# millardjn/rusty_sr

Measured on AMD Instinct MI355X. Metric: output megapixels/sec at 3x upscale (BASELINE '4x'; reference factor is hard-wired 3), higher is better.
Workload: dtype f32

## Files before the change

### rusty_sr_amd/csrc/sr_api.cpp

```cpp
#include <hip/hip_runtime.h>

#include <algorithm>
#include <cmath>
#include <cstdio>
#include <cstdlib>
#include <chrono>
#include <cstring>
#include <new>
#include <string>
#include <thread>
#include <vector>

#include "../../include/srhip.h"
#include "../../include/srhip_experimental.h"
#include "sr_kernels.h"
#include "sr_internal.h"

namespace {

struct ParamLayout {
    size_t conv0, f_bias, f_activ, exp_bias, l_bias[3], l_activ[3], conv1, conv2, conv3, conv5, conv6, conv7, conv8,
        conv9, conv10, end;
    int E;
    explicit ParamLayout(int f) {
// ... 317 lines not shown
        pack_conv0_split(w, params + L.conv0);
        c->off_w0h = push(w);
        for (int split = 0; split < 2; ++split) {
            auto ident = [](int, int j) { return j; };
            auto expand = [&](int nt, int j) { return split ? expand_channel_t(factor, nt, j) : expand_channel(factor, nt, j); };
            const bool h16 = split != 0;
            auto conv = [&](const float* wp, int ks) { if (h16) pack_steps_h16(w, wp, ks); else pack_steps(w, wp, ks, 1, split != 0, ident); };
            auto exp3 = [&](const float* wp) { pack_steps(w, wp, 3, expand_tiles(factor), split != 0, expand); };
            size_t* off = split ? c->off_wh : c->off_w;
            w.clear(); conv(params + L.conv1, 5);
            off[1] = push(w);
            w.clear(); conv(params + L.conv2, 5); conv(params + L.conv5, 3);
            off[2] = push(w);
            w.clear(); conv(params + L.conv3, 5); conv(params + L.conv6, 3); conv(params + L.conv8, 3);
            off[3] = push(w);
            w.clear();
            exp3(params + L.conv7); exp3(params + L.conv9); exp3(params + L.conv10);
            if (split) pack_lin_split(w, factor);
            else pack_lin(w, factor);
            off[4] = push(w);
        }
        w.clear(); pack_steps_wino(w, params + L.conv1);
        c->off_wino1 = push(w);
        const size_t boff[4] = {L.f_bias, L.l_bias[0], L.l_bias[1], L.l_bias[2]};
        const size_t aoff[4] = {L.f_activ, L.l_activ[0], L.l_activ[1], L.l_activ[2]};
        for (int s = 0; s < 4; ++s) c->off_bias[s] = push(vec32(boff[s], 32));
        for (int s = 0; s < 4; ++s) c->off_beta[s] = push(vec32(aoff[s], 32));
        {
            std::vector<float> eb((size_t)expand_tiles(factor) * 32, 0.0f);
            for (int nt = 0; nt < expand_tiles(factor); ++nt)
                for (int j = 0; j < 32; ++j) {
                    const int ch = expand_channel(factor, nt, j);
                    if (ch >= 0) eb[nt * 32 + j] = params[L.exp_bias + ch];
                }
            c->off_bias[4] = push(eb);
        }
        for (size_t k = L.conv1; k < L.end && c->split_ok; ++k) c->split_ok = std::fabs(params[k]) < 65504.0f;
        for (size_t k = L.conv0; k < L.conv0 + 2400 && c->split_ok; ++k) c->split_ok = std::fabs(params[k]) < 65504.0f;
        mark("weight packing (host)");
        HIPCHK(c, hipHostMalloc((void**)&c->h_domain, 64, hipHostMallocMapped));
        *c->h_domain = 0;
        HIPCHK(c, hipHostGetDevicePointer((void**)&c->d_domain, c->h_domain, 0));
        for (auto& w : c->ws) HIPCHK(c, hipMalloc((void**)&w.d_queue, 5 * 8 * sizeof(int)));

        HIPCHK(c, hipMalloc((void**)&c->d_params, host.size() * sizeof(float)));
        mark("hipMalloc x3");
// ... 74 lines not shown
        while (*v) {
            c->env_rows.push_back(atoi(v));
            while (*v && *v != ',') ++v;
            if (*v) ++v;
        }
    } else if (!strcmp(key, "geo")) {
        c->env_geo = strcmp(v, "0") != 0;
    } else if (!strcmp(key, "tail")) {
        c->env_tail = *v ? (float)atof(v) : -1.0f;
    } else if (!strcmp(key, "fork")) {
        c->env_fork = *v ? atoi(v) : -1;
    } else if (!strcmp(key, "forkshare")) {
        c->fork_share = *v ? std::min(0.9, std::max(0.1, atof(v))) : 0.5;
    } else if (!strcmp(key, "forkmin")) {
        c->fork_min_rounds = *v ? atof(v) : 3.5;
    } else if (!strcmp(key, "forktune")) {
        c->fork_autotune = strcmp(v, "0") != 0;
        sr_device_guard restore_device;
        (void)hipSetDevice(c->device);
        sr_fork_tune_clear(c);
    } else if (!strcmp(key, "halo")) {
        c->layer_halos = !strcmp(v, "layers");
    } else if (!strcmp(key, "wino")) {
        c->wino = strcmp(v, "0") != 0;
    } else if (!strcmp(key, "bw")) {
        c->env_bw = *v ? atoi(v) : -1;
    } else {
        return SR_E_INVALID;
    }
    return SR_OK;
}

int sr_get_experiment(sr_ctx* c, const char* key, char* buf, size_t cap) {
    if (!c || !key || !buf || cap == 0) return SR_E_INVALID;
    std::string out;
    if (!strcmp(key, "forktune")) {
        char line[160];
        for (const auto& t : c->fork_tune) {
            snprintf(line, sizeof line, "%dx%d+%d+%d %s %s %s %.4f %.4f\n", t.H, t.W, t.top, t.bot, t.precision == SR_PRECISION_F32 ? "f32" : "split_f16",
                     t.img_u8 ? "u8" : "f32", t.decided < 0 ? "measuring" : (t.decided ? "forked" : "undivided"),
                     t.best[0] < 1e29f ? t.best[0] : 0.f, t.best[1] < 1e29f ? t.best[1] : 0.f);
            out += line;
        }
    } else if (!strcmp(key, "plan")) {
        for (const auto& r : c->plan_rec) out += r.first + (r.second > 1 ? " x" + std::to_string(r.second) : std::string()) + "\n";
    } else {
        return SR_E_INVALID;
// ... 105 lines not shown
    bool mark = false;
    hipStream_t s = nullptr;
    struct Launch { int y0, y1, ty8, ty4, th, grid; bool pipe; } L[5];
    float* feat[4] = {nullptr, nullptr, nullptr, nullptr};
    int prepare();
    int launch(int st) const;
};

int StackJob::prepare() {
    static const int margin[5] = {5, 3, 2, 1, 0};
    tiles_x = (W + 31) / 32;
    const int rc = ensure_features(c, *ws, n, H, W, tiles_x, s);
    if (rc != SR_OK) return rc;
    const int cus = c->cus > 0 ? c->cus : 256;
    const int resident = 2 * cus;
    const bool planar = c->precision == SR_PRECISION_SPLIT_F16;
    for (int k = 0; k < 4; ++k) feat[k] = ws->d_feat[k] + (planar ? (size_t)kFeatPad * ws->pitch * 32 + kFeatPad * 4 : ((size_t)kFeatPad * ws->pitch + kFeatPad) * 32);
    for (int st = 0; st < 5; ++st) {
        Launch& l = L[st];
        l.y0 = layers ? top : std::max(0, top - margin[st]);
        l.y1 = layers ? bot : std::min(H, bot + margin[st]);
        const int rows = l.y1 - l.y0;
        const long tiles8 = (long)n * tiles_x * ((rows + 7) / 8);
        const bool wino8 = st == 1 && c->precision == SR_PRECISION_F32 && c->wino;
        const int forced = (st == 4 && c->factor == 4 && c->precision == SR_PRECISION_SPLIT_F16) ? 4 : c->env_th[st];
        const bool small_launch = tiles8 < 2L * resident;
        const bool split = c->precision == SR_PRECISION_SPLIT_F16;
        const bool one_small_round = small_launch && (long)n * tiles_x * ((rows + 3) / 4) <= resident;
        l.pipe = st > 0 && c->env_pipe != 0 && (c->env_pipe == 2 || !small_launch || split || (st >= 2 && one_small_round));
        l.ty8 = (rows + 7) / 8; l.ty4 = 0;
        if (forced == 4 || (!forced && small_launch && !wino8 && (!split || tiles8 < cus))) {
            l.ty8 = 0; l.ty4 = (rows + 3) / 4;
        } else if (!forced && l.pipe && !small_launch) {
            const double rounds = (double)tiles8 / resident;
            float tail = c->env_tail;
            if (tail < 0.0f) tail = (!split && rounds >= 3.0 && !forked && st != 4) ? 1.0f : 0.0f;
            if (tail > 0.0f) {
                const long per_row = (long)n * tiles_x;
                const int want = (int)((tail * resident + per_row - 1) / per_row);
                l.ty8 = std::max(0, (rows - 4 * want) / 8);
                l.ty4 = std::max(0, (rows - 8 * l.ty8 + 3) / 4);
            }
        }
        if (!forced && l.pipe && !small_launch && !split && l.ty4 == 0 && (double)tiles8 / resident >= 3.0 && rows % 8 >= 1 && rows % 8 <= 4) {
            l.ty8 = rows / 8; l.ty4 = 1;
        }
        if (l.ty8 > 0 && l.ty4 > 0 && (long)n * tiles_x * (l.ty8 + l.ty4) <= resident) {
            l.ty8 = 0; l.ty4 = (rows + 3) / 4;
        }
        l.th = l.ty8 > 0 ? 8 : 4;
        if (!l.pipe && l.ty8 > 0) { l.ty8 = (rows + 7) / 8; l.ty4 = 0; }
        const int ntiles = n * tiles_x * (l.ty8 + l.ty4);
        l.grid = l.pipe ? std::min(ntiles, resident) : ntiles;
    }
    return SR_OK;
}

int StackJob::launch(int st) const {
    const int cus = c->cus > 0 ? c->cus : 256;
// ... 25 lines not shown
            HIPCHK(c, sr_launch_conv0(a, l.th, c->precision, std::min(a.n_tiles, 8 * cus), img_u8, s));
            return SR_OK;
        };
        if (!gate || !gate->ready) return rows(y0, y1);
        const int lo = late_top > 0 ? std::max(y0, late_top + 2) : y0, hi = late_bot > 0 ? std::min(y1, H - late_bot - 2) : y1;
        int rc = lo < hi ? rows(lo, hi) : SR_OK;
        if (rc != SR_OK) return rc;
        if (mark && gate->mark[0]) HIPCHK(c, hipEventRecord(gate->mark[0], s));
        HIPCHK(c, hipStreamWaitEvent(s, gate->ready, 0));
        if (mark && gate->mark[1]) HIPCHK(c, hipEventRecord(gate->mark[1], s));
        if (lo >= hi) return rows(y0, y1);
        rc = rows(y0, lo);
        return rc != SR_OK ? rc : rows(hi, y1);
    }
    StageArgs a{};
    float* f = feat[0]; float* l1 = feat[1]; float* l2 = feat[2]; float* l3 = feat[3];
    a.pitch = ws->pitch; a.img_stride = ws->img_stride;
    switch (st) {
        case 1: a.src[0] = f; a.dst = l1; break;
        case 2: a.src[0] = f; a.src[1] = l1; a.dst = l2; break;
        case 3: a.src[0] = f; a.src[1] = l1; a.src[2] = l2; a.dst = l3; break;
        case 4: a.src[0] = l1; a.src[1] = l2; a.src[2] = l3; a.img = d_img; a.out = d_out; break;
    }
    const bool wino = st == 1 && c->precision == SR_PRECISION_F32 && c->wino;
    a.wpack = P + (c->precision ? c->off_wh[st] : wino ? c->off_wino1 : c->off_w[st]); a.bias = P + c->off_bias[st];
    a.beta = st < 4 ? P + c->off_beta[st] : nullptr;
    a.H = H; a.W = W; a.img_ch = img_ch;
    a.y_begin = y0; a.y_end = y1; a.tiles_x = tiles_x;
    a.n_img = n; a.queue = ws->d_queue + st * 8; a.domain = c->d_domain;
    a.grid[0] = make_tile_grid(8, y0, l.ty8, tiles_x, n, bw);
    a.grid[1] = make_tile_grid(4, y0 + 8 * l.ty8, l.ty4, tiles_x, n, bw);
    if (l.pipe) HIPCHK(c, sr_launch_stage_pipe(st, c->factor, a, c->precision, l.grid, img_u8, out_u8, wino, s));
    else HIPCHK(c, sr_launch_stage(st, c->factor, a, l.th, c->precision, l.grid, img_u8, out_u8, wino, s));
    return SR_OK;
}

}

int sr_run_stack(sr_ctx* c, const void* d_img, bool img_u8, int img_ch, int n, int H, int W, int halo_top,
                 int halo_bot, void* d_out, bool out_u8, hipStream_t s, int slot, const sr_halo_gate* gate) {
    if (!c || !d_img || !d_out || slot < 0 || slot > 1) return SR_E_INVALID;
    sr_device_guard restore_device;
    if (n <= 0 || H <= 0 || W <= 0) return SR_E_INVALID;
    if (img_u8 && img_ch != 3 && img_ch != 4) return SR_E_INVALID;
    if (c->graph != SR_GRAPH_SR_NET) {
        if (halo_top || halo_bot || gate) return SR_E_INVALID;
        if (c->graph == SR_GRAPH_DOWNSAMPLE && (H < 3 || W < 3)) return SR_E_INVALID;
        if (img_u8 != out_u8) return SR_E_INVALID;
// ... 744 lines not shown
```

### rusty_sr_amd/csrc/sr_internal.h

```cpp
#pragma once
#include <hip/hip_runtime.h>

#include <cstdint>
#include <string>
#include <utility>
#include <vector>

#include "../../include/srhip.h"

struct sr_ctx {
    int device = 0;
    int cus = 0, clock_mhz = 0;
    char name[128] = {0};
    hipStream_t stream = nullptr;
    float* d_params = nullptr;
    void* d_qtab = nullptr;
    size_t off_w0 = 0, off_w0h = 0, off_w[5] = {0}, off_wh[5] = {0}, off_bias[5] = {0}, off_beta[5] = {0};
    size_t off_wino1 = 0;
    bool wino = true;
    int precision = 0;
    bool split_ok = true;
    int* h_domain = nullptr;
    int* d_domain = nullptr;
    int domain_fallbacks = 0;
    bool dev_fault = false;
    int graph = SR_GRAPH_SR_NET;
    int factor = SR_FACTOR;
    struct Workspace {
        float* d_feat[4] = {nullptr, nullptr, nullptr, nullptr};
        size_t feat_cap_px = 0;
        int geo_n = 0, geo_h = 0, geo_w = 0;
        int pitch = 0; long img_stride = 0;
        int* d_queue = nullptr;
    } ws[2];
    hipStream_t stream2 = nullptr;
    void* d_in[2] = {nullptr, nullptr};  size_t in_cap[2] = {0, 0};
    void* d_out[2] = {nullptr, nullptr}; size_t out_cap[2] = {0, 0};
    hipStream_t copy_out = nullptr;
    hipStream_t copy_in = nullptr;
    int pipelined_calls = 0;
    std::vector<hipEvent_t> pool;
    int pipeline = 1;
// ... 145 lines not shown
```

### rusty_sr_amd/csrc/sr_kernels.hip

```cpp
#include <hip/hip_runtime.h>
#include <stddef.h>
#include <stdint.h>

#include <mutex>
#include <set>
#include <type_traits>
#include <utility>

#include "sr_kernels.h"

#pragma clang fp contract(off)

typedef float f32x2 __attribute__((ext_vector_type(2)));
struct f32p { float x, y; };
__device__ __forceinline__ f32p operator+(f32p a, f32p b) { return f32p{a.x + b.x, a.y + b.y}; }
__device__ __forceinline__ f32p operator-(f32p a, f32p b) { return f32p{a.x - b.x, a.y - b.y}; }
__device__ __forceinline__ f32p operator*(f32p a, f32p b) { return f32p{a.x * b.x, a.y * b.y}; }
__device__ __forceinline__ f32p p_fma(f32p a, f32p b, f32p c) { return f32p{__builtin_fmaf(a.x, b.x, c.x), __builtin_fmaf(a.y, b.y, c.y)}; }
__device__ __forceinline__ void store_map8(char* p, uint32_t a, uint32_t b) { *(uint2*)p = make_uint2(a, b); }
typedef float f32x4 __attribute__((ext_vector_type(4)));
typedef float f32x16 __attribute__((ext_vector_type(16)));
typedef _Float16 f16x8 __attribute__((ext_vector_type(8)));
typedef _Float16 f16x2 __attribute__((ext_vector_type(2)));

// ... 510 lines not shown
        __builtin_amdgcn_sched_barrier(0);
        cur = nxt;
      }
    }
}

constexpr int kWinoGroups = 5 * 7 * 2;
constexpr int kWinoSteps = (kWinoGroups + 3) / 4;
constexpr int wino_acc(int k) { return k < 4 ? k : k - 3; }
constexpr int wino_ca(int k) { return k == 0 ? 0 : k == 1 ? 1 : k == 2 ? 2 : k == 3 ? 1 : k == 4 ? 3 : k == 5 ? 4 : 3; }
constexpr int wino_cb(int k) { return k == 0 ? 2 : k == 1 ? 2 : k == 2 ? 1 : k == 3 ? 3 : k == 4 ? 4 : k == 5 ? 3 : 5; }
constexpr bool wino_add(int k) { return k == 1 || k == 4; }

template <bool ADD>
__device__ __forceinline__ void wino_u4(f32x2 x0, f32x2 y0, f32x2 x1, f32x2 y1, f32x2& u0, f32x2& u1) {
    if constexpr (ADD)
        asm("v_pk_add_f32 %0, %2, %3\n\tv_pk_add_f32 %1, %4, %5\n\ts_nop 1"
            : "=&v"(u0), "=&v"(u1) : "v"(x0), "v"(y0), "v"(x1), "v"(y1));
    else
        asm("v_pk_add_f32 %0, %2, %3 neg_lo:[0,1] neg_hi:[0,1]\n\tv_pk_add_f32 %1, %4, %5 neg_lo:[0,1] neg_hi:[0,1]\n\ts_nop 1"
            : "=&v"(u0), "=&v"(u1) : "v"(x0), "v"(y0), "v"(x1), "v"(y1));
}

template <int TWH, int PS, int T, typename Stream>
__device__ __forceinline__ void half_steps_wino(f32x16 (&acc)[4], const char* hb, const char* ring, Stream& sm, int wave, int lane) {
    static_assert(TWH >= kTW + 4, "a pair reads six pixels from its first halo column on");
    const int i = lane & 31, h = lane >> 5;
    const int wlane = (h * 32 + i) * 16;
    const int row = wave * T + (T == 2 ? i >> 4 : 0);
    const char* abase = hb + h * PS + (row * TWH + 2 * (i & 15)) * 16;
    struct Ops { f32x4 x, y, b; };
    auto load = [&](Ops& o, int g, int sl) {
        const int rr = g & 1, k = (g >> 1) % 7, ky = (g >> 1) / 7;
        const char* ab = abase + rr * 2 * PS + ky * TWH * 16;
        o.b = *(const f32x4*)(ring + sl * 4096 + wlane + (g & 3) * 1024);
        o.x = *(const f32x4*)(ab + wino_ca(k) * 16);
        o.y = *(const f32x4*)(ab + wino_cb(k) * 16);
    };
    auto mfma = [&](const Ops& o, int g) {
        const int k = (g >> 1) % 7;
        const f32x2 x0 = {o.x[0], o.x[1]}, x1 = {o.x[2], o.x[3]}, y0 = {o.y[0], o.y[1]}, y1 = {o.y[2], o.y[3]};
        f32x2 u0, u1;
        if (wino_add(k)) wino_u4<true>(x0, y0, x1, y1, u0, u1);
        else wino_u4<false>(x0, y0, x1, y1, u0, u1);
        const float u[4] = {u0.x, u0.y, u1.x, u1.y};
#pragma unroll
        for (int e = 0; e < 4; ++e) acc[wino_acc(k)] = __builtin_amdgcn_mfma_f32_32x32x2f32(u[e], o.b[e], acc[wino_acc(k)], 0, 0, 0);
    };
    Ops cur, nxt;
    load(cur, 0, sm.slot());
#pragma unroll
    for (int s = 0; s < kWinoSteps; ++s) {
        const int ngroups = kWinoGroups - 4 * s < 4 ? kWinoGroups - 4 * s : 4;
        sm.begin_step();
#pragma unroll
        for (int q = 0; q < 3; ++q) {
            if (q + 1 < ngroups) {
                load(nxt, 4 * s + q + 1, sm.slot());
                sm.piece(4 * s + q);
                __builtin_amdgcn_sched_barrier(0);
                mfma(cur, 4 * s + q);
                __builtin_amdgcn_sched_barrier(0);
                cur = nxt;
            }
        }
        const bool last = s == kWinoSteps - 1;
        sm.template end_step<0>(last);
        if (!last) load(nxt, 4 * s + 4, sm.slot());
        sm.piece(4 * s + 3);
        __builtin_amdgcn_sched_barrier(0);
        mfma(cur, 4 * s + ngroups - 1);
        __builtin_amdgcn_sched_barrier(0);
        cur = nxt;
    }
}

template <int TWH, int PS, int LO, int KS, int T, int NTN, typename Stream>
__device__ __forceinline__ void half_steps_h(f32x16 (&accm)[NTN * T], f32x16 (&accx)[NTN * T], const char* hb, const char* ring,
                                             Stream& sm, int wave, int lane) {
    constexpr int NT = KS * KS, NP = (NT + 1) / 2;
    const int i = lane & 31, h = lane >> 5;
    const int wlane = (h * 32 + i) * 16;
    const char* abase = hb + h * PS + ((wave * T) * TWH + i) * 16;
    struct Ops { f16x8 bh[2], bl[2], ah[2][T], al[2][T]; };
    auto row_id = [](int p, int ts, int m) {
        const int t = 2 * p + ts;
        return t < NT ? (t / KS) * 16 + (t % KS) + m : -1;
    };
    auto load = [&](Ops& o, const Ops& prev, int pp, int p, int sl) {
        const char* wb = ring + sl * 4096 + wlane;
#pragma unroll
        for (int ts = 0; ts < 2; ++ts) {
            const int t = 2 * p + ts;
            if (t >= NT) continue;
// ... 414 lines not shown
                    };
                    if (full_x) {
                        uint32_t px[16];
#pragma unroll
                        for (int r = 0; r < 16; r += 2) quant2(r, px[r], px[r + 1]);
                        if (writer) for_each_acc_row([&](int r, int row) { base[row * FACTOR] = px[r]; });
                    } else {
#pragma unroll
                        for (int r = 0; r < 16; r += 2) {
                            uint32_t p0, p1;
                            quant2(r, p0, p1);
                            const int row0 = (r & 3) + 8 * (r >> 2);
                            if (writer && x0 + 4 * h + row0 < a.W) base[row0 * FACTOR] = p0;
                            if (writer && x0 + 4 * h + row0 + 1 < a.W) base[(row0 + 1) * FACTOR] = p1;
                        }
                    }
                }
            }
        }
    }
    return stores;
}

template <int T>
__device__ __forceinline__ int stage_epilogue_wino(const StageArgs& a, const f32x16 (&acc)[4], float bias, float beta, int n, int x0, int y0,
                                                   int wave, int lane, float* stage_lds) {
    const int i = lane & 31, h = lane >> 5;
    const bool full_x = x0 + kTW <= a.W;
    int stores = 0;
#pragma unroll
    for (int m = 0; m < T; ++m) {
        const int y = y0 + wave * T + m;
        if (y >= a.y_end) continue;
        float* grow = a.dst + ((size_t)n * a.img_stride + (long)y * a.pitch + x0) * 32;
        float o[16];
#pragma unroll
        for (int k = 0; k < 8; k += 2) {
            const int r = 8 * m + k;
            const f32x2 m0 = {acc[0][r], acc[0][r + 1]}, m1 = {acc[1][r], acc[1][r + 1]};
            const f32x2 m2 = {acc[2][r], acc[2][r + 1]}, m3 = {acc[3][r], acc[3][r + 1]};
            const f32x2 bb = {bias, bias};
            const f32x2 p0 = belu2(((m0 + m1) + m2) + bb, beta), p1 = belu2(((m1 - m2) - m3) + bb, beta);
            o[2 * k] = p0.x; o[2 * k + 1] = p1.x; o[2 * k + 2] = p0.y; o[2 * k + 3] = p1.y;
        }
        auto pixel = [&](int v) { return 2 * (((v >> 1) & 3) + 8 * (v >> 3) + 4 * h) + (v & 1); };
        if (full_x && stage_lds) {
            float* sp = stage_lds + i;
#pragma unroll
            for (int v = 0; v < 16; ++v) sp[pixel(v) * 32] = o[v];
            const f32x4* lp = (const f32x4*)stage_lds + lane;
            const f32x4 v0 = lp[0], v1 = lp[64], v2 = lp[128], v3 = lp[192];
            f32x4* gp = (f32x4*)grow + lane;
            gp[0] = v0; gp[64] = v1; gp[128] = v2; gp[192] = v3;
            stores += 4;
        } else if (full_x) {
#pragma unroll
            for (int v = 0; v < 16; ++v) grow[pixel(v) * 32 + i] = o[v];
            stores += 16;
        } else {
#pragma unroll
            for (int v = 0; v < 16; ++v)
                if (x0 + pixel(v) < a.W) grow[pixel(v) * 32 + i] = o[v];
        }
    }
    return stores;
// ... 187 lines not shown

__device__ __forceinline__ void run_of_xcd(int x, int ntiles, int& start, int& count) {
    const int q = ntiles >> 3, r = ntiles & 7;
    count = q + (x < r ? 1 : 0);
    start = x < r ? x * (q + 1) : r * (q + 1) + (x - r) * q;
}
__device__ __forceinline__ int queue_slot(int x, int nbig, int nsmall, int idx) {
    int start, count;
    run_of_xcd(x, nbig, start, count);
    if (idx < count) return start + idx;
    idx -= count;
    run_of_xcd(x, nsmall, start, count);
    return idx < count ? nbig + start + idx : -1;
}
__device__ __forceinline__ int queue_total(int x, int nbig, int nsmall) {
    int start, cb, cs;
    run_of_xcd(x, nbig, start, cb);
    run_of_xcd(x, nsmall, start, cs);
    return cb + cs;
}
__device__ __forceinline__ int queue_first(int block, int nbig, int nsmall) { return queue_slot(block & 7, nbig, nsmall, block >> 3); }
template <int TH, int NSRC, int KS0, bool FINAL, bool IMG_U8, bool OUT_U8, int PREC, int FACTOR = 3, bool WINO = false>
__global__ __launch_bounds__(256, 2) void conv_stage_kernel(StageArgs a) {
    static_assert(!WINO || (NSRC == 1 && KS0 == 5 && !FINAL && PREC == 0), "WINO: stage 1 of the exact mode");
    __builtin_amdgcn_s_setprio(3);
    constexpr int NW = 4, T = TH / NW;
    constexpr int NTN = FINAL ? (FACTOR * FACTOR + 9) / 10 : 1;
    using G0 = TileGeom<TH, KS0>;
    extern __shared__ __attribute__((aligned(16))) char smem[];
    char* tile = smem;
    char* ring = smem + 8 * G0::PLANE;

    const int tid = threadIdx.x, lane = tid & 63;
    const int wave = __builtin_amdgcn_readfirstlane(tid >> 6);
    const int i = lane & 31;
    constexpr bool H16 = kH16<PREC, FINAL>;
    constexpr int NTAPS = WINO ? 2 * kWinoSteps
                        : H16 ? KS0 * KS0 + (NSRC - 1) * 9
                              : 2 * ((KS0 * KS0 + 1) / 2 + (NSRC - 1) * 5) * NTN;
    const TileGrid& grid = a.grid[TH == 8 ? 0 : 1];
    float bias[NTN];
#pragma unroll
    for (int nt = 0; nt < NTN; ++nt) bias[nt] = a.bias[nt * 32 + i];
    const float beta = FINAL ? 0.f : a.beta[i];

    TileOffsets<TH, KS0, NW> off0;
    TileOffsets<TH, 3, NW> off3;
    off0.template init<PREC>(a.pitch, wave, lane);
    if constexpr (NSRC >= 2) off3.template init<PREC>(a.pitch, wave, lane);
    int n, tx, ty;
    tile_coords(grid, a.tiles_x, xcd_remap(blockIdx.x, gridDim.x), n, tx, ty);
    const int x0 = tx * kTW, y0 = grid.y0 + ty * TH;
#pragma unroll
    for (int k = 0; k < kRingAhead; ++k) weight_chunk_async(ring + k * 4096, a.wpack + k * kChunkFloats, wave, lane);
    stage_tile<TH, KS0, PREC, NW>(tile, a.src[0], off0, a.img_stride, a.pitch, n, y0, x0, wave, lane);

    f32x16 acc[NTN * T], accx[PREC == 1 ? NTN * T : 1];
#pragma unroll
    for (int m = 0; m < NTN * T; ++m)
#pragma unroll
        for (int r = 0; r < 16; ++r) {
            acc[m][r] = (PREC == 1 && !FINAL) ? bias[0] : 0.f;
            if constexpr (PREC == 1) accx[m][r] = 0.f;
        }
    f32x4 qm[H16 ? T : 1][2][2], qx[H16 ? T : 1][2][2];
    f32x4 bias2[2], beta2[2];
    if constexpr (H16) {
#pragma unroll
        for (int ch = 0; ch < 2; ++ch) {
            bias2[ch] = *(const f32x4*)(a.bias + 16 * ch + 4 * (lane >> 4));
            beta2[ch] = *(const f32x4*)(a.beta + 16 * ch + 4 * (lane >> 4));
        }
#pragma unroll
        for (int m = 0; m < T; ++m)
#pragma unroll
            for (int k = 0; k < 4; ++k) { qm[m][k >> 1][k & 1] = bias2[k & 1]; qx[m][k >> 1][k & 1] = f32x4{0.f, 0.f, 0.f, 0.f}; }
    }
    f32x16 wacc[WINO ? 4 : 1];
#pragma unroll
    for (int p = 0; p < (WINO ? 4 : 1); ++p)
#pragma unroll
        for (int r = 0; r < 16; ++r) wacc[p][r] = 0.f;
    int gtap = 0, slot = 0;
    auto taps = [&](auto ks_tag) {
        constexpr int KS = decltype(ks_tag)::value;
        if constexpr (WINO) {
            using G = TileGeom<TH, KS>;
            RingStream sm{ring, a.wpack, gtap, slot, NTAPS, wave, lane};
#pragma unroll 1
            for (int half = 0; half < 2; ++half) half_steps_wino<G::TWH, G::PLANE, T>(wacc, tile + half * 4 * G::PLANE, ring, sm, wave, lane);
        } else if constexpr (H16) source_steps_h16<TH, KS, T>(qm, qx, tile, ring, a.wpack, gtap, slot, NTAPS, wave, lane);
        else source_steps<TH, KS, T, NTN, PREC>(acc, accx, tile, ring, a.wpack, gtap, slot, NTAPS, wave, lane);
    };
    ring_barrier<0>();
    __builtin_amdgcn_s_setprio(0);
    taps(std::integral_constant<int, KS0>{});
    if constexpr (NSRC >= 2) {
        __builtin_amdgcn_s_setprio(3);
        stage_tile<TH, 3, PREC, NW>(tile, a.src[1], off3, a.img_stride, a.pitch, n, y0, x0, wave, lane);
        ring_barrier<0>();
        __builtin_amdgcn_s_setprio(0);
        taps(std::integral_constant<int, 3>{});
    }
    if constexpr (NSRC >= 3) {
        __builtin_amdgcn_s_setprio(3);
        stage_tile<TH, 3, PREC, NW>(tile, a.src[2], off3, a.img_stride, a.pitch, n, y0, x0, wave, lane);
        ring_barrier<0>();
        __builtin_amdgcn_s_setprio(0);
        taps(std::integral_constant<int, 3>{});
    }
    __builtin_amdgcn_s_setprio(3);
    if constexpr (FINAL)
        lin_taps<TH, T, IMG_U8, NW * 64, NTN, PREC, FACTOR>(acc, accx, tile, ring, a, a.wpack + (size_t)NTAPS * kChunkFloats, n, y0, x0, wave, lane, tid);
    uint32_t dom = 0;
    if constexpr (WINO) {
        stage_epilogue_wino<T>(a, wacc, bias[0], beta, n, x0, y0, wave, lane, nullptr);
    } else if constexpr (H16) {
        stage_epilogue_h16<T>(a, qm, qx, beta2, n, x0, y0, wave, lane, dom);
    } else if constexpr (FINAL && PREC == 1) {
        f32x4 fbias[NTN][4];
#pragma unroll
        for (int nt = 0; nt < NTN; ++nt)
#pragma unroll
            for (int k = 0; k < 4; ++k) fbias[nt][k] = *(const f32x4*)(a.bias + 32 * nt + 16 * (lane >> 5) + 4 * k);
        stage_epilogue_final_t<T, NTN, OUT_U8, FACTOR>(a, acc, accx, fbias, n, x0, y0, wave, lane);
    } else {
        static_assert(PREC == 0, "the split-half mode's tiles have epilogues of their own");
        stage_epilogue<TH, T, NTN, FINAL, OUT_U8, FACTOR>(a, acc, bias, beta, n, x0, y0, wave, lane);
    }
    if constexpr (PREC == 1 && !FINAL) domain_report(dom, a.domain);
}

#define SR_WAIT_ROW(k, extra) "s_waitcnt vmcnt(" #k ")" extra "\n\ts_branch .Lsrwait%=\n\t"
#define SR_WAIT_ROWS10(b, extra)                                                                                              \
    SR_WAIT_ROW(b##0, extra) SR_WAIT_ROW(b##1, extra) SR_WAIT_ROW(b##2, extra) SR_WAIT_ROW(b##3, extra) SR_WAIT_ROW(b##4, extra) \
    SR_WAIT_ROW(b##5, extra) SR_WAIT_ROW(b##6, extra) SR_WAIT_ROW(b##7, extra) SR_WAIT_ROW(b##8, extra) SR_WAIT_ROW(b##9, extra)
#define SR_WAIT_JUMP(maxn)                                                                                                   \
    "s_max_i32 %0, %1, 0\n\ts_min_i32 %0, %0, " #maxn "\n\ts_lshl_b32 %0, %0, 3\n\ts_add_u32 %0, %0, 12\n\t"                 \
    "s_getpc_b64 vcc\n\ts_add_u32 vcc_lo, vcc_lo, %0\n\ts_addc_u32 vcc_hi, vcc_hi, 0\n\ts_setpc_b64 vcc\n\t"
// ... 247 lines not shown
    int step_no;
    Hook last_step_hook;
    __device__ __forceinline__ void begin_step() {
        step_request(st, gs0 + step_no, ring_lds, wbase, lane);
        if (mailbox && step_no == snap_step) queue_presolve(a, xcd, wave, lane, st, qs);
        ++step_no;
    }
    __device__ __forceinline__ void piece(int g) {
        if (g < HalfTile<KSN>::G::NG && g < rq.ng) {
            htn.stage_one(g, rq.origin, rq.dst);
            st.tile_seq = ++st.issued;
        }
    }
    __device__ __forceinline__ int slot() const { return st.slot; }
    template <int EXTRA> __device__ __forceinline__ void end_step(bool last) {
        if (last) last_step_hook();
        if (last && mailbox) queue_publish(a, xcd, wave, lane, st, qs, mailbox);
        step_advance<EXTRA>(st, last, PREC == 1 && gs0 + step_no <= kRingAhead);
    }
};

template <int NSRC, int KS0, bool FINAL, bool IMG_U8, bool OUT_U8, int PREC, int FACTOR = 3, bool WINO = false>
__global__ __launch_bounds__(256, 2) void conv_stage_pipe_kernel(StageArgs a) {
    static_assert(!WINO || (NSRC == 1 && KS0 == 5 && !FINAL && PREC == 0), "WINO: stage 1 of the exact mode");
    __builtin_amdgcn_s_setprio(3);
    constexpr int NTN = FINAL ? (FACTOR * FACTOR + 9) / 10 : 1;
    using H0 = HalfTile<KS0>;
    using H3 = HalfTile<3>;
    constexpr int HB = H0::BYTES;
    constexpr int NH = 2 * NSRC;
    constexpr bool H16 = kH16<PREC, FINAL>;
    constexpr int NSTEPS = WINO ? 2 * kWinoSteps
                         : H16 ? KS0 * KS0 + (NSRC - 1) * 9
                               : 2 * (H0::STEPS + (NSRC - 1) * H3::STEPS) * NTN;
    extern __shared__ __attribute__((aligned(16))) char smem[];
    char* ring = smem + 2 * HB;
    volatile int* s_next = (volatile int*)(ring + kRingBytes);
    float* s_wlin = (float*)(ring + kRingBytes + 16);
    float* s_lut = s_wlin + 9 * NTN * 128;
    constexpr bool kLinOwn = FINAL && NTN == 1;
    float* s_xown = s_lut + 256;
    const uint32_t lds0 = lds_addr(smem);

    const int tid = threadIdx.x, lane = tid & 63;
    const int wave = __builtin_amdgcn_readfirstlane(tid >> 6);
    const int i = lane & 31;
    const int nbig = a.grid[0].ntiles, nsmall = a.grid[1].ntiles;
    const int xcd = blockIdx.x & 7;
    const uint32_t ring_lds = __builtin_amdgcn_readfirstlane(lds_addr(ring) + wave * 1024);
    const char* wbase = uniform_ptr((const char*)a.wpack + wave * 1024);
    float bias[NTN];
#pragma unroll
    for (int nt = 0; nt < NTN; ++nt) bias[nt] = a.bias[nt * 32 + i];
    const float beta = FINAL ? 0.f : a.beta[i];
    f32x4 bias2[2], beta2[2];
// ... 70 lines not shown
        f32x16 acc[NTN * T], accx[PREC == 1 ? NTN * T : 1];
#pragma unroll
        for (int m = 0; m < NTN * T; ++m)
#pragma unroll
            for (int r = 0; r < 16; ++r) {
                acc[m][r] = (PREC == 1 && !FINAL) ? bias[0] : 0.f;
                if constexpr (PREC == 1) accx[m][r] = 0.f;
            }
        f32x4 qm[H16 ? T : 1][2][2], qx[H16 ? T : 1][2][2];
        if constexpr (H16) {
#pragma unroll
            for (int m = 0; m < T; ++m)
#pragma unroll
                for (int k = 0; k < 4; ++k) { qm[m][k >> 1][k & 1] = bias2[k & 1]; qx[m][k >> 1][k & 1] = f32x4{0.f, 0.f, 0.f, 0.f}; }
        }
        constexpr bool QUAD = FINAL && PREC == 0 && T == 2;
        QuadAcc qa[QUAD ? NTN : 1];
        if constexpr (QUAD) {
#pragma unroll
            for (int nt = 0; nt < NTN; ++nt)
#pragma unroll
                for (int g = 0; g < 8; ++g) qa[nt][g] = f32x4{0.f, 0.f, 0.f, 0.f};
        }
        f32x16 wacc[WINO ? 4 : 1];
#pragma unroll
        for (int p = 0; p < (WINO ? 4 : 1); ++p)
#pragma unroll
            for (int r = 0; r < 16; ++r) wacc[p][r] = 0.f;
        QueueState qs{0u, 0u, 0, 0, -1};
        if (!single) queue_pull_async(a, xcd, wave, lane, st, qs);
        st.have_next = false;
        LinPrefetch<IMG_U8, TH> linpx;
        auto do_half = [&](auto jc) {
            constexpr int j = decltype(jc)::value;
            constexpr int src = j >> 1;
            constexpr int KSJ = src == 0 ? KS0 : 3;
            constexpr int KSN = (j + 1 < NH) ? (((j + 1) >> 1) == 0 ? KS0 : 3) : KS0;
            const uint32_t other = lds0 + ((j + 1) & 1) * HB;
            const char* hb = smem + (j & 1) * HB;
            if constexpr (j == 1) {
                const int next = single ? -1 : __builtin_amdgcn_readfirstlane(*s_next);
                st.have_next = next >= 0;
                if (st.have_next) coords(next, nn, nx0, ny0, nsmall_tile);
            }
            HalfRequest rq;
            if constexpr (j + 1 < NH)
                rq = HalfRequest{T == 2 ? HalfTile<KSN>::G::NG : HalfTile<KSN>::NG_SMALL,
                                 HalfTile<KSN>::template origin_of<PREC>(a.src[(j + 1) >> 1], (j + 1) & 1, a.img_stride, a.pitch, n, y0, x0, wave),
                                 HalfTile<KSN>::plane_of(other, wave)};
            else
                rq = HalfRequest{!st.have_next ? 0 : nsmall_tile ? HalfTile<KSN>::NG_SMALL : HalfTile<KSN>::G::NG,
                                 HalfTile<KSN>::template origin_of<PREC>(a.src[0], 0, a.img_stride, a.pitch, nn, ny0, nx0, wave),
                                 HalfTile<KSN>::plane_of(other, wave)};
            if constexpr (FINAL && j == (kLinOwn ? NH - 2 : NH - 1)) linpx.issue(a, n, y0, x0, tid, st);
            const HalfTile<KSN>* htn;
            if constexpr (KSN == KS0) htn = (const HalfTile<KSN>*)&h0; else htn = (const HalfTile<KSN>*)&h3;
            using GJ = TileGeom<8, KSJ>;
            constexpr int PAIRS_J = (KSJ * KSJ - 1) / 2;
            constexpr int STEPS_J = WINO ? kWinoSteps : H16 ? PAIRS_J + (j & 1) : HalfTile<KSJ>::STEPS * NTN;
            constexpr int GS0 = WINO ? j * kWinoSteps : H16 ? (src == 0 ? 0 : KS0 * KS0 + (src - 1) * 9) + (j & 1) * PAIRS_J
                                    : (j == 0 ? 0 : j == 1 ? H0::STEPS : 2 * H0::STEPS + (j - 2) * H3::STEPS) * NTN;
            constexpr int LIN_LO_J = LinPrefetch<IMG_U8, TH>::NPIX * 8;
            auto lin_store = [&]() {
                if constexpr (kLinOwn && j == NH - 2) {
                    if constexpr (PREC == 1) linpx.store_split((char*)s_xown, LIN_LO_J, (const uint32_t*)s_lut, 4.0f * FACTOR * FACTOR, tid, st);
                    else linpx.store(s_xown, s_lut, tid, st);
                    asm volatile("s_waitcnt lgkmcnt(0)" ::: "memory");
                }
            };
            PipeStream<PREC, KSN, decltype(lin_store)> sm{st, rq, *htn, a, ring_lds, wbase, GS0, wave, lane, (j == 0 && !single) ? s_next : nullptr, xcd, qs, STEPS_J > 3 ? STEPS_J - 3 : 0, 0, lin_store};
            if constexpr (WINO) half_steps_wino<GJ::TWH, GJ::PLANE, T>(wacc, hb, ring, sm, wave, lane);
            else if constexpr (QUAD) half_steps_f32<GJ::TWH, GJ::PLANE, KSJ, T, NTN, true, FACTOR>(qa, hb, ring, sm, wave, lane);
            else if constexpr (PREC == 0) half_steps_f32<GJ::TWH, GJ::PLANE, KSJ, T, NTN>(acc, hb, ring, sm, wave, lane);
            else if constexpr (H16) half_steps_h16<GJ::TWH, GJ::PLANE, 2, KSJ, T, (j & 1) != 0, -HB>(qm, qx, hb, ring, sm, wave, lane);
            else half_steps_h<GJ::TWH, GJ::PLANE, 2, KSJ, T, NTN>(acc, accx, hb, ring, sm, wave, lane);
        };
        do_half(std::integral_constant<int, 0>{});
        do_half(std::integral_constant<int, 1>{});
        if constexpr (NH > 2) { do_half(std::integral_constant<int, 2>{}); do_half(std::integral_constant<int, 3>{}); }
        if constexpr (NH > 4) { do_half(std::integral_constant<int, 4>{}); do_half(std::integral_constant<int, 5>{}); }
        if constexpr (FINAL) {
            constexpr int LIN_LO = LinPrefetch<IMG_U8, TH>::NPIX * 8;
            float* s_x = kLinOwn ? s_xown : (float*)(smem + HB);
            if constexpr (!kLinOwn) {
                if constexpr (PREC == 1) linpx.store_split((char*)s_x, LIN_LO, (const uint32_t*)s_lut, 4.0f * FACTOR * FACTOR, tid, st);
                else linpx.store(s_x, s_lut, tid, st);
                asm volatile("s_waitcnt lgkmcnt(0)" ::: "memory");
                __builtin_amdgcn_s_barrier();
                asm volatile("" ::: "memory");
            }
            if constexpr (PREC == 1) lin_mfma_h<TH, T, NTN>(acc, accx, (const char*)s_x, LIN_LO, (const f16x8*)s_wlin, wave, lane);
            else if constexpr (QUAD) lin_mfma_quad<NTN, FACTOR>(qa, s_x, s_wlin, wave, lane);
            else lin_mfma<TH, T, NTN>(acc, s_x, s_wlin, wave, lane);
            if constexpr (!kLinOwn) {
                asm volatile("s_waitcnt lgkmcnt(0)" ::: "memory");
                __builtin_amdgcn_s_barrier();
                asm volatile("" ::: "memory");
            }
        }
        int stores;
        if constexpr (H16) stores = stage_epilogue_h16<T>(a, qm, qx, beta2, n, x0, y0, wave, lane, dom);
        else if constexpr (QUAD) stores = stage_epilogue_quad<NTN, OUT_U8, FACTOR>(a, qa, qbias, n, x0, y0, wave, lane);
        else if constexpr (kFinalT) stores = stage_epilogue_final_t<T, NTN, OUT_U8, FACTOR>(a, acc, accx, fbias, n, x0, y0, wave, lane);
        else {
            float* scratch = FINAL ? nullptr : (float*)(smem + ((NH - 1) & 1) * HB + wave * H0::G::PLANE);
            if constexpr (WINO) stores = stage_epilogue_wino<T>(a, wacc, bias[0], beta, n, x0, y0, wave, lane, scratch);
            else stores = stage_epilogue<TH, T, NTN, FINAL, OUT_U8, FACTOR>(a, acc, bias, beta, n, x0, y0, wave, lane, scratch);
        }
        if constexpr (PREC == 1) st.issued += stores;
    };

    constexpr bool kBigTiles = !(FINAL && FACTOR == 4 && PREC == 1);
    int budget = nbig + nsmall;
    while (true) {
        if constexpr (kBigTiles) {
            if (small) tile_body(std::integral_constant<int, 1>{});
            else tile_body(std::integral_constant<int, 2>{});
        } else {
            if (!small) __builtin_trap();
            tile_body(std::integral_constant<int, 1>{});
        }
        if (!st.have_next) break;
        if (--budget <= 0) {
            asm volatile("s_waitcnt vmcnt(0)" ::: "memory");
            __builtin_trap();
        }
        n = nn; x0 = nx0; y0 = ny0; small = nsmall_tile;
    }
    if constexpr (PREC == 1 && !FINAL) domain_report(dom, a.domain);
// ... 68 lines not shown
    hipError_t e = hipGetDevice(&dev);
    if (e != hipSuccess) return e;
    {
        std::lock_guard<std::mutex> lock(mu);
        const auto key = std::make_pair((const void*)kern, dev);
        if (!configured.count(key)) {
            e = hipFuncSetAttribute((const void*)kern, hipFuncAttributeMaxDynamicSharedMemorySize, (int)lds);
            if (e != hipSuccess) return e;
            configured.insert(key);
        }
    }
    hipLaunchKernelGGL(kern, dim3(nblk), dim3(kThreads), lds, s, a);
    return hipGetLastError();
}

template <int TH, int PREC>
static hipError_t launch_stage_t(int stage, int factor, const StageArgs& a, int nblk, bool img_u8, bool out_u8, bool wino,
                                 hipStream_t s) {
    switch (stage) {
        case 1:
            if constexpr (PREC == 0)
                if (wino) return launch_with_lds(conv_stage_kernel<TH, 1, 5, false, false, false, 0, 3, true>, a, nblk, stage_lds_bytes<TH, 5>(), s);
            return launch_with_lds(conv_stage_kernel<TH, 1, 5, false, false, false, PREC>, a, nblk, stage_lds_bytes<TH, 5>(), s);
        case 2: return launch_with_lds(conv_stage_kernel<TH, 2, 5, false, false, false, PREC>, a, nblk, stage_lds_bytes<TH, 5>(), s);
        case 3: return launch_with_lds(conv_stage_kernel<TH, 3, 5, false, false, false, PREC>, a, nblk, stage_lds_bytes<TH, 5>(), s);
        case 4:
#define SR_FINAL(F)                                                                                                          \
            if (img_u8 && out_u8) return launch_with_lds(conv_stage_kernel<TH, 3, 3, true, true, true, PREC, F>, a, nblk, stage_lds_bytes<TH, 3>(), s); \
            if (!img_u8 && !out_u8) return launch_with_lds(conv_stage_kernel<TH, 3, 3, true, false, false, PREC, F>, a, nblk, stage_lds_bytes<TH, 3>(), s); \
            return hipErrorInvalidValue;
            if (factor == 3) { SR_FINAL(3) }
            if (factor == 2) { SR_FINAL(2) }
            if (factor == 4) { SR_FINAL(4) }
#undef SR_FINAL
            return hipErrorInvalidValue;
        default: return hipErrorInvalidValue;
    }
}

template <int PREC>
static hipError_t launch_stage_pipe_t(int stage, int factor, const StageArgs& a, int grid, bool img_u8, bool out_u8, bool wino, hipStream_t s) {
    constexpr size_t lds5 = 2 * (size_t)HalfTile<5>::BYTES + kRingBytes + 16;
    constexpr size_t lds3_1 = 2 * (size_t)HalfTile<3>::BYTES + kRingBytes + 16 + 9 * 128 * sizeof(float) + 256 * sizeof(float) + 10 * 34 * 16;
    constexpr size_t lds3_2 = 2 * (size_t)HalfTile<3>::BYTES + kRingBytes + 16 + 9 * 2 * 128 * sizeof(float) + 256 * sizeof(float);
    static_assert(lds3_1 <= 80 * 1024 && lds3_2 <= 80 * 1024, "two workgroups per CU");
    const size_t lds3 = factor == 4 ? lds3_2 : lds3_1;
    switch (stage) {
        case 1:
            if constexpr (PREC == 0)
                if (wino) return launch_with_lds(conv_stage_pipe_kernel<1, 5, false, false, false, 0, 3, true>, a, grid, lds5, s);
            return launch_with_lds(conv_stage_pipe_kernel<1, 5, false, false, false, PREC>, a, grid, lds5, s);
        case 2: return launch_with_lds(conv_stage_pipe_kernel<2, 5, false, false, false, PREC>, a, grid, lds5, s);
        case 3: return launch_with_lds(conv_stage_pipe_kernel<3, 5, false, false, false, PREC>, a, grid, lds5, s);
        case 4:
#define SR_FINAL(F)                                                                                                          \
            if (img_u8 && out_u8) return launch_with_lds(conv_stage_pipe_kernel<3, 3, true, true, true, PREC, F>, a, grid, lds3, s); \
            if (!img_u8 && !out_u8) return launch_with_lds(conv_stage_pipe_kernel<3, 3, true, false, false, PREC, F>, a, grid, lds3, s); \
            return hipErrorInvalidValue;
            if (factor == 3) { SR_FINAL(3) }
            if (factor == 2) { SR_FINAL(2) }
            if (factor == 4) { SR_FINAL(4) }
#undef SR_FINAL
            return hipErrorInvalidValue;
    }
    return hipErrorInvalidValue;
}
hipError_t sr_launch_stage_pipe(int stage, int factor, const StageArgs& a, int prec, int grid, bool img_u8, bool out_u8, bool wino, hipStream_t s) {
    return prec == 0 ? launch_stage_pipe_t<0>(stage, factor, a, grid, img_u8, out_u8, wino, s)
                     : launch_stage_pipe_t<1>(stage, factor, a, grid, img_u8, out_u8, wino, s);
}

hipError_t sr_launch_stage(int stage, int factor, const StageArgs& a, int th, int prec, int nblk, bool img_u8,
                           bool out_u8, bool wino, hipStream_t s) {
    if (prec == 0)
        return th == 8 ? launch_stage_t<8, 0>(stage, factor, a, nblk, img_u8, out_u8, wino, s)
// ... 5 lines not shown
```

Before: 5017.

## Extend Winograd-style path to stage 2 with a pairwise 3x3 source

Extends the Winograd-style exact f32 convolution path, previously used only for stage 1, to stage 2. The 5x5 source uses the existing Winograd steps, and the second 3x3 source uses a new pairwise-tap MFMA routine that accumulates into a fifth accumulator, which is folded into the odd-pixel output during the epilogue. The goal is fewer MFMA and weight-streaming steps for stage 2. The cost is more accumulator registers, a new weight pack, and turning off the tail split for this stage. The wino setting becomes an integer that defaults to enabling both stages.

```diff
diff --git a/rusty_sr_amd/csrc/sr_api.cpp b/rusty_sr_amd/csrc/sr_api.cpp
--- a/rusty_sr_amd/csrc/sr_api.cpp
+++ b/rusty_sr_amd/csrc/sr_api.cpp
@@ -363,6 +363,8 @@
         }
         w.clear(); pack_steps_wino(w, params + L.conv1);
         c->off_wino1 = push(w);
+        w.clear(); pack_steps_wino(w, params + L.conv2); pack_steps(w, params + L.conv5, 3, 1, false, [](int, int j) { return j; });
+        c->off_wino2 = push(w);
         const size_t boff[4] = {L.f_bias, L.l_bias[0], L.l_bias[1], L.l_bias[2]};
         const size_t aoff[4] = {L.f_activ, L.l_activ[0], L.l_activ[1], L.l_activ[2]};
         for (int s = 0; s < 4; ++s) c->off_bias[s] = push(vec32(boff[s], 32));
@@ -483,7 +485,7 @@
     } else if (!strcmp(key, "halo")) {
         c->layer_halos = !strcmp(v, "layers");
     } else if (!strcmp(key, "wino")) {
-        c->wino = strcmp(v, "0") != 0;
+        c->wino = !strcmp(v, "0") ? 0 : !strcmp(v, "1") ? 1 : 2;
     } else if (!strcmp(key, "bw")) {
         c->env_bw = *v ? atoi(v) : -1;
     } else {
@@ -635,7 +637,7 @@
         l.y1 = layers ? bot : std::min(H, bot + margin[st]);
         const int rows = l.y1 - l.y0;
         const long tiles8 = (long)n * tiles_x * ((rows + 7) / 8);
-        const bool wino8 = st == 1 && c->precision == SR_PRECISION_F32 && c->wino;
+        const bool wino8 = c->precision == SR_PRECISION_F32 && (st == 1 || st == 2) && st <= c->wino;
         const int forced = (st == 4 && c->factor == 4 && c->precision == SR_PRECISION_SPLIT_F16) ? 4 : c->env_th[st];
         const bool small_launch = tiles8 < 2L * resident;
         const bool split = c->precision == SR_PRECISION_SPLIT_F16;
@@ -647,7 +649,7 @@
         } else if (!forced && l.pipe && !small_launch) {
             const double rounds = (double)tiles8 / resident;
             float tail = c->env_tail;
-            if (tail < 0.0f) tail = (!split && rounds >= 3.0 && !forked && st != 4) ? 1.0f : 0.0f;
+            if (tail < 0.0f) tail = (!split && rounds >= 3.0 && !forked && st != 4 && !(st == 2 && wino8)) ? 1.0f : 0.0f;
             if (tail > 0.0f) {
                 const long per_row = (long)n * tiles_x;
                 const int want = (int)((tail * resident + per_row - 1) / per_row);
@@ -719,8 +721,8 @@
         case 3: a.src[0] = f; a.src[1] = l1; a.src[2] = l2; a.dst = l3; break;
         case 4: a.src[0] = l1; a.src[1] = l2; a.src[2] = l3; a.img = d_img; a.out = d_out; break;
     }
-    const bool wino = st == 1 && c->precision == SR_PRECISION_F32 && c->wino;
-    a.wpack = P + (c->precision ? c->off_wh[st] : wino ? c->off_wino1 : c->off_w[st]); a.bias = P + c->off_bias[st];
+    const bool wino = c->precision == SR_PRECISION_F32 && (st == 1 || st == 2) && st <= c->wino;
+    a.wpack = P + (c->precision ? c->off_wh[st] : !wino ? c->off_w[st] : st == 1 ? c->off_wino1 : c->off_wino2); a.bias = P + c->off_bias[st];
     a.beta = st < 4 ? P + c->off_beta[st] : nullptr;
     a.H = H; a.W = W; a.img_ch = img_ch;
     a.y_begin = y0; a.y_end = y1; a.tiles_x = tiles_x;
diff --git a/rusty_sr_amd/csrc/sr_internal.h b/rusty_sr_amd/csrc/sr_internal.h
--- a/rusty_sr_amd/csrc/sr_internal.h
+++ b/rusty_sr_amd/csrc/sr_internal.h
@@ -17,7 +17,8 @@
     void* d_qtab = nullptr;
     size_t off_w0 = 0, off_w0h = 0, off_w[5] = {0}, off_wh[5] = {0}, off_bias[5] = {0}, off_beta[5] = {0};
     size_t off_wino1 = 0;
-    bool wino = true;
+    size_t off_wino2 = 0;
+    int wino = 2;
     int precision = 0;
     bool split_ok = true;
     int* h_domain = nullptr;
diff --git a/rusty_sr_amd/csrc/sr_kernels.hip b/rusty_sr_amd/csrc/sr_kernels.hip
--- a/rusty_sr_amd/csrc/sr_kernels.hip
+++ b/rusty_sr_amd/csrc/sr_kernels.hip
@@ -556,8 +556,8 @@
             : "=&v"(u0), "=&v"(u1) : "v"(x0), "v"(y0), "v"(x1), "v"(y1));
 }
 
-template <int TWH, int PS, int T, typename Stream>
-__device__ __forceinline__ void half_steps_wino(f32x16 (&acc)[4], const char* hb, const char* ring, Stream& sm, int wave, int lane) {
+template <int TWH, int PS, int T, int NA, typename Stream>
+__device__ __forceinline__ void half_steps_wino(f32x16 (&acc)[NA], const char* hb, const char* ring, Stream& sm, int wave, int lane) {
     static_assert(TWH >= kTW + 4, "a pair reads six pixels from its first halo column on");
     const int i = lane & 31, h = lane >> 5;
     const int wlane = (h * 32 + i) * 16;
@@ -604,6 +604,57 @@
         sm.piece(4 * s + 3);
         __builtin_amdgcn_sched_barrier(0);
         mfma(cur, 4 * s + ngroups - 1);
+        __builtin_amdgcn_sched_barrier(0);
+        cur = nxt;
+    }
+}
+
+template <int TWH, int PS, int T, typename Stream>
+__device__ __forceinline__ void half_steps_pairs(f32x16 (&acc)[5], const char* hb, const char* ring, Stream& sm, int wave, int lane) {
+    constexpr int NT = 9, NP = (NT + 1) / 2;
+    static_assert(TWH >= kTW + 2, "a pair reads four pixels from its first halo column on");
+    const int i = lane & 31, h = lane >> 5;
+    const int wlane = (h * 32 + i) * 16;
+    const int row = wave * T + (T == 2 ? i >> 4 : 0);
+    const char* abase = hb + h * PS + (row * TWH + 2 * (i & 15)) * 16;
+    struct Ops { f32x4 x, y, b; };
+    auto load = [&](Ops& o, int p, int q, int sl) {
+        const int t = 2 * p + (q >> 1), ky = t / 3, kx = t - ky * 3;
+        const char* ab = abase + (q & 1) * 2 * PS + (ky * TWH + kx) * 16;
+        o.b = *(const f32x4*)(ring + sl * 4096 + wlane + q * 1024);
+        o.x = *(const f32x4*)ab;
+        o.y = *(const f32x4*)(ab + 16);
+    };
+    auto mfma = [&](const Ops& o) {
+#pragma unroll
+        for (int e = 0; e < 4; ++e) {
+            acc[0] = __builtin_amdgcn_mfma_f32_32x32x2f32(o.x[e], o.b[e], acc[0], 0, 0, 0);
+            acc[4] = __builtin_amdgcn_mfma_f32_32x32x2f32(o.y[e], o.b[e], acc[4], 0, 0, 0);
+        }
+    };
+    Ops cur, nxt;
+    load(cur, 0, 0, sm.slot());
+#pragma unroll
+    for (int p = 0; p < NP; ++p) {
+        const int ngroups = (2 * p + 1 < NT) ? 4 : 2;
+        sm.begin_step();
+#pragma unroll
+        for (int q = 0; q < 3; ++q) {
+            if (q + 1 < ngroups) {
+                load(nxt, p, q + 1, sm.slot());
+                sm.piece(4 * p + q);
+                __builtin_amdgcn_sched_barrier(0);
+                mfma(cur);
+                __builtin_amdgcn_sched_barrier(0);
+                cur = nxt;
+            }
+        }
+        const bool last = p == NP - 1;
+        sm.template end_step<0>(last);
+        if (!last) load(nxt, p + 1, 0, sm.slot());
+        sm.piece(4 * p + 3);
+        __builtin_amdgcn_sched_barrier(0);
+        mfma(cur);
         __builtin_amdgcn_sched_barrier(0);
         cur = nxt;
     }
@@ -1064,9 +1115,10 @@
     return stores;
 }
 
-template <int T>
-__device__ __forceinline__ int stage_epilogue_wino(const StageArgs& a, const f32x16 (&acc)[4], float bias, float beta, int n, int x0, int y0,
+template <int T, int NA>
+__device__ __forceinline__ int stage_epilogue_wino(const StageArgs& a, const f32x16 (&acc)[NA], float bias, float beta, int n, int x0, int y0,
                                                    int wave, int lane, float* stage_lds) {
+    static_assert(NA == 4 || NA == 5, "four position sets, or four and stage 2's odd-pixel set");
     const int i = lane & 31, h = lane >> 5;
     const bool full_x = x0 + kTW <= a.W;
     int stores = 0;
@@ -1082,7 +1134,9 @@
             const f32x2 m0 = {acc[0][r], acc[0][r + 1]}, m1 = {acc[1][r], acc[1][r + 1]};
             const f32x2 m2 = {acc[2][r], acc[2][r + 1]}, m3 = {acc[3][r], acc[3][r + 1]};
             const f32x2 bb = {bias, bias};
-            const f32x2 p0 = belu2(((m0 + m1) + m2) + bb, beta), p1 = belu2(((m1 - m2) - m3) + bb, beta);
+            f32x2 y1 = (m1 - m2) - m3;
+            if constexpr (NA == 5) y1 = y1 + f32x2{acc[4][r], acc[4][r + 1]};
+            const f32x2 p0 = belu2(((m0 + m1) + m2) + bb, beta), p1 = belu2(y1 + bb, beta);
             o[2 * k] = p0.x; o[2 * k + 1] = p1.x; o[2 * k + 2] = p0.y; o[2 * k + 3] = p1.y;
         }
         auto pixel = [&](int v) { return 2 * (((v >> 1) & 3) + 8 * (v >> 3) + 4 * h) + (v & 1); };
@@ -1316,7 +1370,7 @@
 __device__ __forceinline__ int queue_first(int block, int nbig, int nsmall) { return queue_slot(block & 7, nbig, nsmall, block >> 3); }
 template <int TH, int NSRC, int KS0, bool FINAL, bool IMG_U8, bool OUT_U8, int PREC, int FACTOR = 3, bool WINO = false>
 __global__ __launch_bounds__(256, 2) void conv_stage_kernel(StageArgs a) {
-    static_assert(!WINO || (NSRC == 1 && KS0 == 5 && !FINAL && PREC == 0), "WINO: stage 1 of the exact mode");
+    static_assert(!WINO || (NSRC <= 2 && KS0 == 5 && !FINAL && PREC == 0), "WINO: stages 1 and 2 of the exact mode");
     __builtin_amdgcn_s_setprio(3);
     constexpr int NW = 4, T = TH / NW;
     constexpr int NTN = FINAL ? (FACTOR * FACTOR + 9) / 10 : 1;
@@ -1329,7 +1383,7 @@
     const int wave = __builtin_amdgcn_readfirstlane(tid >> 6);
     const int i = lane & 31;
     constexpr bool H16 = kH16<PREC, FINAL>;
-    constexpr int NTAPS = WINO ? 2 * kWinoSteps
+    constexpr int NTAPS = WINO ? 2 * (kWinoSteps + (NSRC - 1) * 5)
                         : H16 ? KS0 * KS0 + (NSRC - 1) * 9
                               : 2 * ((KS0 * KS0 + 1) / 2 + (NSRC - 1) * 5) * NTN;
     const TileGrid& grid = a.grid[TH == 8 ? 0 : 1];
@@ -1370,9 +1424,10 @@
 #pragma unroll
             for (int k = 0; k < 4; ++k) { qm[m][k >> 1][k & 1] = bias2[k & 1]; qx[m][k >> 1][k & 1] = f32x4{0.f, 0.f, 0.f, 0.f}; }
     }
-    f32x16 wacc[WINO ? 4 : 1];
-#pragma unroll
-    for (int p = 0; p < (WINO ? 4 : 1); ++p)
+    constexpr int NWACC = WINO ? 3 + NSRC : 1;
+    f32x16 wacc[NWACC];
+#pragma unroll
+    for (int p = 0; p < NWACC; ++p)
 #pragma unroll
         for (int r = 0; r < 16; ++r) wacc[p][r] = 0.f;
     int gtap = 0, slot = 0;
@@ -1382,7 +1437,10 @@
             using G = TileGeom<TH, KS>;
             RingStream sm{ring, a.wpack, gtap, slot, NTAPS, wave, lane};
 #pragma unroll 1
-            for (int half = 0; half < 2; ++half) half_steps_wino<G::TWH, G::PLANE, T>(wacc, tile + half * 4 * G::PLANE, ring, sm, wave, lane);
+            for (int half = 0; half < 2; ++half) {
+                if constexpr (KS == KS0) half_steps_wino<G::TWH, G::PLANE, T>(wacc, tile + half * 4 * G::PLANE, ring, sm, wave, lane);
+                else half_steps_pairs<G::TWH, G::PLANE, T>(wacc, tile + half * 4 * G::PLANE, ring, sm, wave, lane);
+            }
         } else if constexpr (H16) source_steps_h16<TH, KS, T>(qm, qx, tile, ring, a.wpack, gtap, slot, NTAPS, wave, lane);
         else source_steps<TH, KS, T, NTN, PREC>(acc, accx, tile, ring, a.wpack, gtap, slot, NTAPS, wave, lane);
     };
@@ -1408,7 +1466,7 @@
         lin_taps<TH, T, IMG_U8, NW * 64, NTN, PREC, FACTOR>(acc, accx, tile, ring, a, a.wpack + (size_t)NTAPS * kChunkFloats, n, y0, x0, wave, lane, tid);
     uint32_t dom = 0;
     if constexpr (WINO) {
-        stage_epilogue_wino<T>(a, wacc, bias[0], beta, n, x0, y0, wave, lane, nullptr);
+        stage_epilogue_wino<T, NWACC>(a, wacc, bias[0], beta, n, x0, y0, wave, lane, nullptr);
     } else if constexpr (H16) {
         stage_epilogue_h16<T>(a, qm, qx, beta2, n, x0, y0, wave, lane, dom);
     } else if constexpr (FINAL && PREC == 1) {
@@ -1702,7 +1760,7 @@
 
 template <int NSRC, int KS0, bool FINAL, bool IMG_U8, bool OUT_U8, int PREC, int FACTOR = 3, bool WINO = false>
 __global__ __launch_bounds__(256, 2) void conv_stage_pipe_kernel(StageArgs a) {
-    static_assert(!WINO || (NSRC == 1 && KS0 == 5 && !FINAL && PREC == 0), "WINO: stage 1 of the exact mode");
+    static_assert(!WINO || (NSRC <= 2 && KS0 == 5 && !FINAL && PREC == 0), "WINO: stages 1 and 2 of the exact mode");
     __builtin_amdgcn_s_setprio(3);
     constexpr int NTN = FINAL ? (FACTOR * FACTOR + 9) / 10 : 1;
     using H0 = HalfTile<KS0>;
@@ -1710,7 +1768,7 @@
     constexpr int HB = H0::BYTES;
     constexpr int NH = 2 * NSRC;
     constexpr bool H16 = kH16<PREC, FINAL>;
-    constexpr int NSTEPS = WINO ? 2 * kWinoSteps
+    constexpr int NSTEPS = WINO ? 2 * (kWinoSteps + (NSRC - 1) * H3::STEPS)
                          : H16 ? KS0 * KS0 + (NSRC - 1) * 9
                                : 2 * (H0::STEPS + (NSRC - 1) * H3::STEPS) * NTN;
     extern __shared__ __attribute__((aligned(16))) char smem[];
@@ -1827,9 +1885,10 @@
 #pragma unroll
                 for (int g = 0; g < 8; ++g) qa[nt][g] = f32x4{0.f, 0.f, 0.f, 0.f};
         }
-        f32x16 wacc[WINO ? 4 : 1];
-#pragma unroll
-        for (int p = 0; p < (WINO ? 4 : 1); ++p)
+        constexpr int NWACC = WINO ? 3 + NSRC : 1;
+        f32x16 wacc[NWACC];
+#pragma unroll
+        for (int p = 0; p < NWACC; ++p)
 #pragma unroll
             for (int r = 0; r < 16; ++r) wacc[p][r] = 0.f;
         QueueState qs{0u, 0u, 0, 0, -1};
@@ -1862,8 +1921,8 @@
             if constexpr (KSN == KS0) htn = (const HalfTile<KSN>*)&h0; else htn = (const HalfTile<KSN>*)&h3;
             using GJ = TileGeom<8, KSJ>;
             constexpr int PAIRS_J = (KSJ * KSJ - 1) / 2;
-            constexpr int STEPS_J = WINO ? kWinoSteps : H16 ? PAIRS_J + (j & 1) : HalfTile<KSJ>::STEPS * NTN;
-            constexpr int GS0 = WINO ? j * kWinoSteps : H16 ? (src == 0 ? 0 : KS0 * KS0 + (src - 1) * 9) + (j & 1) * PAIRS_J
+            constexpr int STEPS_J = WINO ? (src == 0 ? kWinoSteps : H3::STEPS) : H16 ? PAIRS_J + (j & 1) : HalfTile<KSJ>::STEPS * NTN;
+            constexpr int GS0 = WINO ? (j < 2 ? j * kWinoSteps : 2 * kWinoSteps + (j - 2) * H3::STEPS) : H16 ? (src == 0 ? 0 : KS0 * KS0 + (src - 1) * 9) + (j & 1) * PAIRS_J
                                     : (j == 0 ? 0 : j == 1 ? H0::STEPS : 2 * H0::STEPS + (j - 2) * H3::STEPS) * NTN;
             constexpr int LIN_LO_J = LinPrefetch<IMG_U8, TH>::NPIX * 8;
             auto lin_store = [&]() {
@@ -1874,7 +1933,8 @@
                 }
             };
             PipeStream<PREC, KSN, decltype(lin_store)> sm{st, rq, *htn, a, ring_lds, wbase, GS0, wave, lane, (j == 0 && !single) ? s_next : nullptr, xcd, qs, STEPS_J > 3 ? STEPS_J - 3 : 0, 0, lin_store};
-            if constexpr (WINO) half_steps_wino<GJ::TWH, GJ::PLANE, T>(wacc, hb, ring, sm, wave, lane);
+            if constexpr (WINO && src == 0) half_steps_wino<GJ::TWH, GJ::PLANE, T>(wacc, hb, ring, sm, wave, lane);
+            else if constexpr (WINO) half_steps_pairs<GJ::TWH, GJ::PLANE, T>(wacc, hb, ring, sm, wave, lane);
             else if constexpr (QUAD) half_steps_f32<GJ::TWH, GJ::PLANE, KSJ, T, NTN, true, FACTOR>(qa, hb, ring, sm, wave, lane);
             else if constexpr (PREC == 0) half_steps_f32<GJ::TWH, GJ::PLANE, KSJ, T, NTN>(acc, hb, ring, sm, wave, lane);
             else if constexpr (H16) half_steps_h16<GJ::TWH, GJ::PLANE, 2, KSJ, T, (j & 1) != 0, -HB>(qm, qx, hb, ring, sm, wave, lane);
@@ -1909,7 +1969,7 @@
         else if constexpr (kFinalT) stores = stage_epilogue_final_t<T, NTN, OUT_U8, FACTOR>(a, acc, accx, fbias, n, x0, y0, wave, lane);
         else {
             float* scratch = FINAL ? nullptr : (float*)(smem + ((NH - 1) & 1) * HB + wave * H0::G::PLANE);
-            if constexpr (WINO) stores = stage_epilogue_wino<T>(a, wacc, bias[0], beta, n, x0, y0, wave, lane, scratch);
+            if constexpr (WINO) stores = stage_epilogue_wino<T, NWACC>(a, wacc, bias[0], beta, n, x0, y0, wave, lane, scratch);
             else stores = stage_epilogue<TH, T, NTN, FINAL, OUT_U8, FACTOR>(a, acc, bias, beta, n, x0, y0, wave, lane, scratch);
         }
         if constexpr (PREC == 1) st.issued += stores;
@@ -2024,7 +2084,10 @@
             if constexpr (PREC == 0)
                 if (wino) return launch_with_lds(conv_stage_kernel<TH, 1, 5, false, false, false, 0, 3, true>, a, nblk, stage_lds_bytes<TH, 5>(), s);
             return launch_with_lds(conv_stage_kernel<TH, 1, 5, false, false, false, PREC>, a, nblk, stage_lds_bytes<TH, 5>(), s);
-        case 2: return launch_with_lds(conv_stage_kernel<TH, 2, 5, false, false, false, PREC>, a, nblk, stage_lds_bytes<TH, 5>(), s);
+        case 2:
+            if constexpr (PREC == 0)
+                if (wino) return launch_with_lds(conv_stage_kernel<TH, 2, 5, false, false, false, 0, 3, true>, a, nblk, stage_lds_bytes<TH, 5>(), s);
+            return launch_with_lds(conv_stage_kernel<TH, 2, 5, false, false, false, PREC>, a, nblk, stage_lds_bytes<TH, 5>(), s);
         case 3: return launch_with_lds(conv_stage_kernel<TH, 3, 5, false, false, false, PREC>, a, nblk, stage_lds_bytes<TH, 5>(), s);
         case 4:
 #define SR_FINAL(F)                                                                                                          \
@@ -2052,7 +2115,10 @@
             if constexpr (PREC == 0)
                 if (wino) return launch_with_lds(conv_stage_pipe_kernel<1, 5, false, false, false, 0, 3, true>, a, grid, lds5, s);
             return launch_with_lds(conv_stage_pipe_kernel<1, 5, false, false, false, PREC>, a, grid, lds5, s);
-        case 2: return launch_with_lds(conv_stage_pipe_kernel<2, 5, false, false, false, PREC>, a, grid, lds5, s);
+        case 2:
+            if constexpr (PREC == 0)
+                if (wino) return launch_with_lds(conv_stage_pipe_kernel<2, 5, false, false, false, 0, 3, true>, a, grid, lds5, s);
+            return launch_with_lds(conv_stage_pipe_kernel<2, 5, false, false, false, PREC>, a, grid, lds5, s);
         case 3: return launch_with_lds(conv_stage_pipe_kernel<3, 5, false, false, false, PREC>, a, grid, lds5, s);
         case 4:
 #define SR_FINAL(F)                                                                                                          \
```

Result: faster. 5273, median of 6 (+5.1%).
